# BolinLai/CSTS

Hardware: AMD Instinct MI355X
Metric: clips/sec training (fwd+bwd) CSTS-Ego4D 16x256^2 bf16 (higher is better)
Workload: dtype bf16; 1 GPU; CSTS_Ego4D_Gaze_Forecast.yaml train step (fwd + KLDiv + 0.05*EgoNCE + bwd + clip + AdamW), 16x256^2 video + 24 kHz STFT audio, b=4/GPU; mode=train, global_batch=4, frames=16, crop=256, parallelism=dp1, step=hip_graph, hip_graph=True, rccl_ranks=1

## Files before the change

### csts_amd/csrc/attention.hip

```cpp
#include <type_traits>
#include <utility>
#include "common.h"

#ifndef CSTS_ATTN_PART
#define CSTS_ATTN_PART 0
#endif
#ifndef CSTS_DKV_DEPTH
#define CSTS_DKV_DEPTH 4
#endif
#ifndef CSTS_DKV_SWZ
#define CSTS_DKV_SWZ 0
#endif

#ifdef CSTS_ATTN_STAMPS
#if CSTS_ATTN_PART == 1
__device__ unsigned long long g_attn_stamps[4096];
#else
static __device__ unsigned long long g_attn_stamps[4096];
#endif
#define AT_STAMP() do { if (stamp_on && nstamp < 4000) g_attn_stamps[nstamp++] = (unsigned long long)__builtin_amdgcn_s_memtime(); } while (0)
#if CSTS_ATTN_PART == 1
extern "C" int csts_debug_attn_stamps(unsigned long long* dst_host) {
  return (int)hipMemcpyFromSymbol(dst_host, HIP_SYMBOL(g_attn_stamps), sizeof(unsigned long long) * 4096);
}
// ... 863 lines not shown

  tile_loop_dma<HD, KBLK, LD, false>(smem, p.K, kbase, p.k_ts, p.V, vbase, p.v_ts, 0, p.Nk, tid,
                                     [&](const bf16* Ks, const bf16* Vs, int) {
    constexpr int NS = HD / 16, ND = HD / 32, SCB = 2 * NS, PVB = 2 * ND, DEPTH = 4, NBLK = 2 * KT, TOTAL = KT * (SCB + PVB);
    typedef __attribute__((address_space(3))) s16x4 lds_s16x4;
    const int g1 = (lane >> 4) & 1, qq = (lane & 15) >> 2, pp = lane & 3;
    const bf16* rowK = Ks + (lane & 31) * LD + 8 * h;
    const bf16* rowV = Vs + (lane & 31) * LD + 8 * h;
    const bf16* trK = Ks + (4 * h + qq) * LD + 16 * g1 + 4 * pp;
    auto blk_pv = [](int bi) constexpr { return bi == NBLK - 1 || (bi >= 2 && (bi & 1) == 0); };
    auto blk_unit = [](int bi) constexpr { return bi == 0 ? 0 : bi == NBLK - 1 ? KT - 1 : (bi & 1) ? (bi + 1) / 2 : bi / 2 - 1; };
    auto blk_of = [=](int g) constexpr { int bi = 0, s0 = 0; for (;; ++bi) { const int n = blk_pv(bi) ? PVB : SCB; if (g < s0 + n) return bi; s0 += n; } };
    auto blk_start = [=](int bi) constexpr { int s0 = 0; for (int i = 0; i < bi; ++i) s0 += blk_pv(i) ? PVB : SCB; return s0; };
    bf16x8 ring[DEPTH + 1];
    auto request = [&](auto gc) {
      constexpr int g = decltype(gc)::value, bi = blk_of(g), u = blk_unit(bi), k = g - blk_start(bi);
      bf16x8& dst = ring[g % (DEPTH + 1)];
      if constexpr (!blk_pv(bi)) {
        dst = *reinterpret_cast<const bf16x8*>((k < NS ? rowK : rowV) + u * 32 * LD + 16 * (k % NS));
      } else {
        constexpr int s2 = k / ND, d = k % ND;
        const bf16* Yb = trK + (u * 32 + 16 * s2) * LD + 32 * d;
        const bf16x4 b0 = __builtin_bit_cast(bf16x4, __builtin_amdgcn_ds_read_tr16_b64_v4i16((lds_s16x4*)(Yb)));
        const bf16x4 b1 = __builtin_bit_cast(bf16x4, __builtin_amdgcn_ds_read_tr16_b64_v4i16((lds_s16x4*)(Yb + 8 * LD)));
        dst[0] = b0[0]; dst[1] = b0[1]; dst[2] = b0[2]; dst[3] = b0[3];
        dst[4] = b1[0]; dst[5] = b1[1]; dst[6] = b1[2]; dst[7] = b1[3];
      }
    };
    static_for<DEPTH>([&](auto gc) { request(gc); });
    f32x16 S[2], dP[2];
    bf16x8 bp[2][2];
    auto piece = [&](auto suc, auto qc) {
      constexpr int sp = decltype(suc)::value & 1, q = decltype(qc)::value;
#pragma unroll
      for (int r = 2 * q; r < 2 * q + 2; ++r) {
        const float ds = __builtin_amdgcn_exp2f(__builtin_fmaf(S[sp][r], p.scale_log2, negL)) * (dP[sp][r] - dl);
        bp[sp][r / 8][r % 8] = (bf16)ds;
      }
    };
    static_for<TOTAL>([&](auto gc) {
      constexpr int g = decltype(gc)::value, bi = blk_of(g), u = blk_unit(bi), k = g - blk_start(bi), par = u & 1;
      constexpr bool is_pv = blk_pv(bi);
      if constexpr (!is_pv && k == 0) {
#pragma unroll
        for (int r = 0; r < 16; ++r) { S[par][r] = 0.f; dP[par][r] = 0.f; }
      }
      if constexpr (g + DEPTH < TOTAL) request(std::integral_constant<int, g + DEPTH>{});
      const bf16x8 a = ring[g % (DEPTH + 1)];
      if constexpr (!is_pv) {
        if constexpr (k < NS) S[par] = CSTS_MFMA16(a, qf.b[k], S[par], 0, 0, 0);
        else dP[par] = CSTS_MFMA16(a, dof.b[k - NS], dP[par], 0, 0, 0);
      } else {
        constexpr int s2 = k / ND, d = k % ND;
        acc[d] = CSTS_MFMA16(a, bp[par][s2], acc[d], 0, 0, 0);
      }
      if constexpr (bi == 1) {
        if constexpr (k < 8) piece(std::integral_constant<int, 0>{}, std::integral_constant<int, k>{});
      } else if constexpr (bi >= 2 && (bi & 1) == 0) {
        constexpr int su = bi / 2;
        if constexpr (k < 4) piece(std::integral_constant<int, su>{}, std::integral_constant<int, k>{});
        else {
          piece(std::integral_constant<int, su>{}, std::integral_constant<int, 4 + 2 * (k - 4)>{});
          piece(std::integral_constant<int, su>{}, std::integral_constant<int, 5 + 2 * (k - 4)>{});
        }
      }
      __builtin_amdgcn_sched_barrier(0);
    });
  });
  stage_rows_out<HD>(smem, p.dQ, (int64_t)b * p.dq_bs + (int64_t)head * p.dq_hs, p.dq_ts, BX * 128, p.Nq, acc, p.scale,
                     w * 32 + (lane & 31), h, tid);
}

template <int HD, bool F32, bool SLOW>
__global__ __launch_bounds__(256) void attn_dkv_kernel(AttnP p) {
  typedef typename El<F32>::T T;
  typedef Cfg<HD, F32> C;
  constexpr bool FAST = !F32 && HD == 96 && !SLOW;
  constexpr bool SWZ = FAST && (CSTS_DKV_SWZ != 0);
  constexpr int LDF = SWZ ? 128 : C::LD_ROW;
  constexpr int QBLK = FAST ? 128 : C::KVBLK, QT = QBLK / 32;
  extern __shared__ __attribute__((aligned(16))) char smem_raw[];
  T* smem = reinterpret_cast<T*>(smem_raw);
  const int tid = threadIdx.x, lane = tid & 63, w = tid >> 6, h = lane >> 5;
  int BX, BY, BZ;
  xcd_remap3(BX, BY, BZ);
  const int b = BZ / p.H, head = BZ % p.H;
  const int split = BY;
  const int kraw = BX * 128 + w * 32 + (lane & 31);
  const bool kvalid = kraw < p.Nk;
  const int ki = kvalid ? kraw : p.Nk - 1;

  RowFrag<HD, F32> kf, vf;
  kf.load(p.K, (int64_t)b * p.k_bs + (int64_t)ki * p.k_ts + (int64_t)head * p.k_hs, h);
  vf.load(p.V, (int64_t)b * p.v_bs + (int64_t)ki * p.v_ts + (int64_t)head * p.v_hs, h);
  f32x16 dK[HD / 32], dV[HD / 32];
#pragma unroll
  for (int d = 0; d < HD / 32; ++d)
#pragma unroll
    for (int r = 0; r < 16; ++r) { dK[d][r] = 0.f; dV[d][r] = 0.f; }
  const int64_t qbase = (int64_t)b * p.q_bs + (int64_t)head * p.q_hs;
  const int64_t dobase = (int64_t)b * p.do_bs + (int64_t)head * p.do_hs;
  const int qbeg = split * p.q_chunk, qend = min(p.Nq, qbeg + p.q_chunk);
  const float* Lrow = p.LSE + ((int64_t)b * p.H + head) * p.Nq;
  const float* Drow = p.delta + ((int64_t)b * p.H + head) * p.Nq;
  const int fk = frame_of(p, ki);
#ifdef CSTS_ATTN_STAMPS
  const bool stamp_on = tid == 0 && BX == 0 && BY == 0 && BZ == 0;
  int nstamp = 1;
  const unsigned long long rt0 = (unsigned long long)__builtin_amdgcn_s_memrealtime();
#endif
  AT_STAMP();

  auto tile_body = [&](const T* Qs, const T* dOs, int q0, const float* Ls, auto&& dma) {
    const float* Ds = Ls + QBLK;
    AT_STAMP();
    auto softmax_bwd = [&](f32x16& S, f32x16& dP, int qt, int r0, int n) {
      const int j = r0 >> 2, qo = qt * 32 + 8 * j + 4 * h;
      const float4 L4 = *reinterpret_cast<const float4*>(Ls + qo), D4 = *reinterpret_cast<const float4*>(Ds + qo);
      const float l[4] = {L4.x, L4.y, L4.z, L4.w}, dd[4] = {D4.x, D4.y, D4.z, D4.w};
#pragma unroll
      for (int r = r0; r < r0 + n; ++r) {
        const int i = r & 3;
        const float e = __builtin_amdgcn_exp2f(__builtin_fmaf(S[r], p.scale_log2, -l[i]));
        float pr = e;
        if constexpr (SLOW) {
          const int q = q0 + qo + i;
          const bool dead = (q >= qend) | ((p.mask_mode != 0) & (frame_of(p, q) != fk));
          pr = dead ? 0.f : e;
        }
        S[r] = pr;
        dP[r] = pr * (dP[r] - dd[i]);
      }
    };
    if constexpr (F32 || HD != 96) {
#pragma unroll
      for (int qt = 0; qt < QT; ++qt) {
        f32x16 S, dP;
#pragma unroll
        for (int r = 0; r < 16; ++r) { S[r] = 0.f; dP[r] = 0.f; }
        score<HD, C::LD_ROW, F32>(S, Qs + qt * 32 * C::LD_ROW, kf, lane);
        score<HD, C::LD_ROW, F32>(dP, dOs + qt * 32 * C::LD_ROW, vf, lane);
#pragma unroll
        for (int j = 0; j < 4; ++j) softmax_bwd(S, dP, qt, 4 * j, 4);
        pv<HD, C::LD_ROW, F32>(dV, dOs + qt * 32 * C::LD_ROW, S, lane);
        pv<HD, C::LD_ROW, F32>(dK, Qs + qt * 32 * C::LD_ROW, dP, lane);
      }
    } else {
      constexpr int LD = LDF, NS = HD / 16, ND = HD / 32, BLK = 2 * NS, DEPTH = CSTS_DKV_DEPTH, NBLK = 2 * QT, TOTAL = BLK * NBLK;
      static_assert(BLK == 4 * ND, "S/dP and dV/dK blocks have the same number of slots");
      static_assert(QT >= 2, "the block order needs two units");
      typedef __attribute__((address_space(3))) s16x4 lds_s16x4;
      const int g1 = (lane >> 4) & 1, qq = (lane & 15) >> 2, pp = lane & 3;
      constexpr int DOFF = QBLK * LD;
      int rowo[NS], tro[ND][2];
#pragma unroll
      for (int k = 0; k < NS; ++k)
        rowo[k] = (lane & 31) * LD + (SWZ ? (((2 * k + h) ^ swz16(lane & 15)) * 8) : (16 * k + 8 * h));
#pragma unroll
      for (int d = 0; d < ND; ++d)
#pragma unroll
        for (int rd = 0; rd < 2; ++rd) {
          const int row = 4 * h + qq + 8 * rd;
          tro[d][rd] = row * LD + (SWZ ? ((((4 * d + 2 * g1 + (pp >> 1)) ^ swz16(row)) * 8) + 4 * (pp & 1)) : (32 * d + 16 * g1 + 4 * pp));
        }
      bf16x8 ring[DEPTH + 1];
      auto blk_pv = [](int bi) constexpr { return bi == NBLK - 1 || (bi >= 2 && (bi & 1) == 0); };
      auto blk_unit = [](int bi) constexpr { return bi == 0 ? 0 : bi == NBLK - 1 ? QT - 1 : (bi & 1) ? (bi + 1) / 2 : bi / 2 - 1; };
      auto hp_slot = [](int u, int j) constexpr {
        const int w0 = (u == 0 ? BLK : u == QT - 1 ? BLK * (NBLK - 2) : BLK * 2 * u) + 1;
        const int n = ((u == 0 || u == QT - 1) ? BLK : 2 * BLK) - 1;
        return w0 + j * n / 16;
      };
      auto request = [&](auto gc) {
        constexpr int g = decltype(gc)::value, bi = g / BLK, k = g % BLK;
        constexpr bool is_pv = blk_pv(bi);
        constexpr int u = blk_unit(bi);
        bf16x8& dst = ring[g % (DEPTH + 1)];
        if constexpr (!is_pv) {
          dst = *reinterpret_cast<const bf16x8*>(Qs + rowo[k % NS] + (k < NS ? 0 : DOFF) + u * 32 * LD);
        } else {
          constexpr int idx = k % (2 * ND), s2 = idx / ND, d = idx % ND;
          const bf16* Yb = Qs + (k < 2 * ND ? DOFF : 0) + (u * 32 + 16 * s2) * LD;
          const bf16x4 b0 = __builtin_bit_cast(bf16x4, __builtin_amdgcn_ds_read_tr16_b64_v4i16((lds_s16x4*)(Yb + tro[d][0])));
          const bf16x4 b1 = __builtin_bit_cast(bf16x4, __builtin_amdgcn_ds_read_tr16_b64_v4i16((lds_s16x4*)(Yb + tro[d][1])));
          dst[0] = b0[0]; dst[1] = b0[1]; dst[2] = b0[2]; dst[3] = b0[3];
          dst[4] = b1[0]; dst[5] = b1[1]; dst[6] = b1[2]; dst[7] = b1[3];
        }
      };
      static_for<DEPTH>([&](auto gc) { request(gc); });
      f32x16 S[2], dP[2];
      bf16x8 bpS[2][2], bpD[2][2];
      float4 Lq[2][4], Dq[2][4];
      auto comp = [](const float4& v, int i) { return i == 0 ? v.x : i == 1 ? v.y : i == 2 ? v.z : v.w; };
      auto half_piece = [&](auto uc, auto jc) {
        constexpr int u = decltype(uc)::value, j = decltype(jc)::value, sp = u & 1, r0 = 2 * (j / 2), quad = r0 >> 2;
        if constexpr ((j & 1) == 0) {
#pragma unroll
          for (int r = r0; r < r0 + 2; ++r) {
            float e = __builtin_amdgcn_exp2f(__builtin_fmaf(S[sp][r], p.scale_log2, -comp(Lq[sp][quad], r & 3)));
            if constexpr (SLOW) {
              const int q = q0 + u * 32 + 8 * quad + 4 * h + (r & 3);
              const bool dead = (q >= qend) | ((p.mask_mode != 0) & (frame_of(p, q) != fk));
              e = dead ? 0.f : e;
            }
            S[sp][r] = e;
          }
        } else {
#pragma unroll
          for (int r = r0; r < r0 + 2; ++r) dP[sp][r] = S[sp][r] * (dP[sp][r] - comp(Dq[sp][quad], r & 3));
          constexpr int s2 = r0 / 8, e0 = r0 % 8;
          bpS[sp][s2][e0] = (bf16)S[sp][r0]; bpS[sp][s2][e0 + 1] = (bf16)S[sp][r0 + 1];
          bpD[sp][s2][e0] = (bf16)dP[sp][r0]; bpD[sp][s2][e0 + 1] = (bf16)dP[sp][r0 + 1];
        }
      };
      constexpr int NDMA = tile_dma_count<QBLK, LD>();
      static_for<TOTAL>([&](auto gc) {
        constexpr int g = decltype(gc)::value, bi = g / BLK, k = g % BLK;
        constexpr bool is_pv = blk_pv(bi);
        constexpr int u = blk_unit(bi), par = u & 1;
        if constexpr (k == 0) { AT_STAMP(); }
        if constexpr (!is_pv && k == 0) {
#pragma unroll
          for (int r = 0; r < 16; ++r) { S[par][r] = 0.f; dP[par][r] = 0.f; }
        }
        if constexpr (!is_pv && k < 8) {
          const int qo = u * 32 + 8 * (k & 3) + 4 * h;
          if constexpr (k < 4) Lq[par][k] = *reinterpret_cast<const float4*>(Ls + qo);
          else Dq[par][k - 4] = *reinterpret_cast<const float4*>(Ds + qo);
        }
#ifndef CSTS_DKV_DIAG_NOREAD
        if constexpr (g + DEPTH < TOTAL) request(std::integral_constant<int, g + DEPTH>{});
#endif
        const bf16x8 a = ring[g % (DEPTH + 1)];
        if constexpr (!is_pv) {
          if constexpr (k < NS) S[par] = CSTS_MFMA16(a, kf.b[k], S[par], 0, 0, 0);
          else dP[par] = CSTS_MFMA16(a, vf.b[k - NS], dP[par], 0, 0, 0);
        } else {
          constexpr int idx = k % (2 * ND), s2 = idx / ND, d = idx % ND;
#if defined(CSTS_DKV_DIAG_BFRAG) || defined(CSTS_DKV_DIAG_BZERO)
          asm volatile("" ::"v"(bpS[par][s2]), "v"(bpD[par][s2]));
#endif
#ifdef CSTS_DKV_DIAG_BFRAG
          if constexpr (k < 2 * ND) dV[d] = CSTS_MFMA16(a, kf.b[s2 + 2 * par], dV[d], 0, 0, 0);
          else dK[d] = CSTS_MFMA16(a, vf.b[s2 + 2 * par], dK[d], 0, 0, 0);
#elif defined(CSTS_DKV_DIAG_BZERO)
          bf16x8 zz;
#pragma unroll
          for (int e = 0; e < 8; ++e) zz[e] = (bf16)0.f;
          asm volatile("" : "+v"(zz));
          if constexpr (k < 2 * ND) dV[d] = CSTS_MFMA16(a, zz, dV[d], 0, 0, 0);
          else dK[d] = CSTS_MFMA16(a, zz, dK[d], 0, 0, 0);
#else
          if constexpr (k < 2 * ND) dV[d] = CSTS_MFMA16(a, bpS[par][s2], dV[d], 0, 0, 0);
          else dK[d] = CSTS_MFMA16(a, bpD[par][s2], dK[d], 0, 0, 0);
#endif
        }
#ifdef CSTS_DKV_DIAG_NOSM
        if constexpr (!is_pv && k == BLK - 1) asm volatile("" ::"v"(S[par]), "v"(dP[par]));
#endif
#ifndef CSTS_DKV_DIAG_NOSM
        static_for<QT * 16>([&](auto ic) {
          constexpr int i = decltype(ic)::value, su = i / 16, j = i % 16;
          if constexpr (hp_slot(su, j) == g) half_piece(std::integral_constant<int, su>{}, std::integral_constant<int, j>{});
        });
#endif
#ifndef CSTS_DKV_DIAG_NODMA
        if constexpr (g < NDMA) dma(std::integral_constant<int, g>{});
#endif
        __builtin_amdgcn_sched_barrier(0);
      });
    }
    AT_STAMP();
  };
  if constexpr (FAST)
    tile_loop_dma<HD, QBLK, LDF, true, LDF, true, SWZ>(smem, p.Q, qbase, p.q_ts, p.dO, dobase, p.do_ts, qbeg, qend, tid, tile_body,
                                                       Lrow, Drow AT_STAMP_ARGS);
  else
    tile_loop<HD, QBLK, C::LD_ROW, C::LD_ROW, F32, true>(smem, p.Q, qbase, p.q_ts, p.dO, dobase, p.do_ts, qbeg, qend, tid,
                                                         [&](const T* Qs, const T* dOs, int q0, const float* Ls) {
                                                           tile_body(Qs, dOs, q0, Ls, [](auto) {});
                                                         }, Lrow, Drow AT_STAMP_ARGS);
  AT_STAMP();
#ifdef CSTS_ATTN_STAMPS
  if (stamp_on) {
    g_attn_stamps[0] = nstamp;
    g_attn_stamps[4095] = (unsigned long long)__builtin_amdgcn_s_memrealtime() - rt0;
  }
#endif
  if (!kvalid) return;
  if (p.nsplit == 1) {
    store_rows<HD>(p.dK, p.dt, (int64_t)b * p.dk_bs + (int64_t)ki * p.dk_ts + (int64_t)head * p.dk_hs, dK, p.scale, h);
    store_rows<HD>(p.dV, p.dt, (int64_t)b * p.dv_bs + (int64_t)ki * p.dv_ts + (int64_t)head * p.dv_hs, dV, 1.f, h);
  } else {
    const int64_t per = (int64_t)p.B * p.H * p.Nk * HD;
    const int64_t off = (((int64_t)split * p.B + b) * p.H + head) * (int64_t)p.Nk * HD + (int64_t)ki * HD;
    store_rows<HD>(p.ws, CSTS_F32, off, dK, p.scale, h);
    store_rows<HD>(p.ws, CSTS_F32, (int64_t)p.nsplit * per + off, dV, 1.f, h);
  }
}

template <int HD>
__global__ __launch_bounds__(256) void attn_bwd_fused_kernel(AttnP p) {
  typedef Cfg<HD, false> C;
  constexpr int LD = C::LD_ROW, TILE = 128 * LD;
  __shared__ __attribute__((aligned(16))) bf16 smem[5 * TILE + 512];
  bf16* Ks = smem;
  bf16* Vs = smem + TILE;
  bf16* Qs = smem + 2 * TILE;
  bf16* dOs = smem + 3 * TILE;
  bf16* Os = smem + 4 * TILE;
  float* Ls = reinterpret_cast<float*>(smem + 5 * TILE);
  float* Ds = Ls + 128;
  const int tid = threadIdx.x, lane = tid & 63, w = tid >> 6, h = lane >> 5;
  int BX, BY, BZ;
  xcd_remap3(BX, BY, BZ);
  const int b = BY / p.H, head = BY % p.H;
  const int split = BX;
  const int qbeg = split * p.q_chunk, qend = min(p.Nq, qbeg + p.q_chunk);
  const int64_t kbase = (int64_t)b * p.k_bs + (int64_t)head * p.k_hs, vbase = (int64_t)b * p.v_bs + (int64_t)head * p.v_hs;
  const int64_t qbase = (int64_t)b * p.q_bs + (int64_t)head * p.q_hs, dobase = (int64_t)b * p.do_bs + (int64_t)head * p.do_hs;
  const int64_t obase = (int64_t)b * p.o_bs + (int64_t)head * p.o_hs;
  {
    TileStage<HD, 128> sk, sv;
    sk.gload(p.K, kbase, p.k_ts, 0, p.Nk, tid);
    sv.gload(p.V, vbase, p.v_ts, 0, p.Nk, tid);
    sk.lstore(Ks, LD, tid);
    sv.lstore(Vs, LD, tid);
  }

  const int kraw = w * 32 + (lane & 31);
  const bool kvalid = kraw < p.Nk;
  const int ki = kvalid ? kraw : p.Nk - 1;
  RowFrag<HD, false> kf, vf;
  kf.load(p.K, kbase + (int64_t)ki * p.k_ts, h);
  vf.load(p.V, vbase + (int64_t)ki * p.v_ts, h);
  f32x16 dK[HD / 32], dV[HD / 32];
#pragma unroll
  for (int d = 0; d < HD / 32; ++d)
#pragma unroll
    for (int r = 0; r < 16; ++r) { dK[d][r] = 0.f; dV[d][r] = 0.f; }
  const float* Lrow = p.LSE + ((int64_t)b * p.H + head) * p.Nq;

  TileStage<HD, 128> sq, sdo, so;
  float lnext = 0.f;
  sq.gload(p.Q, qbase, p.q_ts, qbeg, qend, tid);
  sdo.gload(p.dO, dobase, p.do_ts, qbeg, qend, tid);
  so.gload(p.O, obase, p.o_ts, qbeg, qend, tid);
  if (tid < 128) lnext = Lrow[min(qbeg + tid, qend - 1)];
  for (int q0 = qbeg; q0 < qend; q0 += 128) {
    __syncthreads();
    sq.lstore(Qs, LD, tid);
    sdo.lstore(dOs, LD, tid);
    so.lstore(Os, LD, tid);
    if (tid < 128) Ls[tid] = lnext;
    if (q0 + 128 < qend) {
      sq.gload(p.Q, qbase, p.q_ts, q0 + 128, qend, tid);
      sdo.gload(p.dO, dobase, p.do_ts, q0 + 128, qend, tid);
      so.gload(p.O, obase, p.o_ts, q0 + 128, qend, tid);
      if (tid < 128) lnext = Lrow[min(q0 + 128 + tid, qend - 1)];
    }
    __syncthreads();
    f32x16 acc[HD / 32];
#pragma unroll
    for (int d = 0; d < HD / 32; ++d)
#pragma unroll
      for (int r = 0; r < 16; ++r) acc[d][r] = 0.f;
    {
      const int qrow = w * 32 + (lane & 31);
      RowFrag<HD, false> qf, dof;
      frag_from_lds<HD>(qf, Qs, qrow, h);
      frag_from_lds<HD>(dof, dOs, qrow, h);
      float dl = 0.f;
      {
        RowFrag<HD, false> of;
        frag_from_lds<HD>(of, Os, qrow, h);
#pragma unroll
        for (int s2 = 0; s2 < HD / 16; ++s2)
#pragma unroll
          for (int j2 = 0; j2 < 8; ++j2) dl += (float)dof.b[s2][j2] * (float)of.b[s2][j2];
      }
      dl += __shfl_xor(dl, 32, 64);
      if (h == 0) Ds[qrow] = dl;
      const float negL = -Ls[qrow];
#pragma unroll
      for (int kt = 0; kt < 4; ++kt) {
        if (kt * 32 >= p.Nk) break;
        f32x16 S, dP;
#pragma unroll
        for (int r = 0; r < 16; ++r) { S[r] = 0.f; dP[r] = 0.f; }
        score<HD, LD, false>(S, Ks + kt * 32 * LD, qf, lane);
        score<HD, LD, false>(dP, Vs + kt * 32 * LD, dof, lane);
#pragma unroll
        for (int r = 0; r < 16; ++r) {
          const float e = __builtin_amdgcn_exp2f(__builtin_fmaf(S[r], p.scale_log2, negL));
          const float pr = (kt * 32 + rowoff(r, h) >= p.Nk) ? 0.f : e;
          S[r] = pr * (dP[r] - dl);
        }
        pv<HD, LD, false>(acc, Ks + kt * 32 * LD, S, lane);
      }
    }
    stage_rows_out_wave<HD>(Os, p.dQ, (int64_t)b * p.dq_bs + (int64_t)head * p.dq_hs, p.dq_ts, q0, qend, acc, p.scale, w, lane);
    __syncthreads();
    const bool ragged = q0 + 128 > qend;
#pragma unroll
    for (int qt = 0; qt < 4; ++qt) {
      f32x16 S, dP;
#pragma unroll
      for (int r = 0; r < 16; ++r) { S[r] = 0.f; dP[r] = 0.f; }
      score<HD, LD, false>(S, Qs + qt * 32 * LD, kf, lane);
      score<HD, LD, false>(dP, dOs + qt * 32 * LD, vf, lane);
#pragma unroll
      for (int j = 0; j < 4; ++j) {
        const int qo = qt * 32 + 8 * j + 4 * h;
        const float4 L4 = *reinterpret_cast<const float4*>(Ls + qo), D4 = *reinterpret_cast<const float4*>(Ds + qo);
        const float l[4] = {L4.x, L4.y, L4.z, L4.w}, dd[4] = {D4.x, D4.y, D4.z, D4.w};
#pragma unroll
        for (int i = 0; i < 4; ++i) {
          const float e = __builtin_amdgcn_exp2f(__builtin_fmaf(S[4 * j + i], p.scale_log2, -l[i]));
          const float pr = (ragged && q0 + qo + i >= qend) ? 0.f : e;
          S[4 * j + i] = pr;
          dP[4 * j + i] = pr * (dP[4 * j + i] - dd[i]);
        }
      }
      pv<HD, LD, false>(dV, dOs + qt * 32 * LD, S, lane);
      pv<HD, LD, false>(dK, Qs + qt * 32 * LD, dP, lane);
    }
  }
  if (!kvalid) return;
  if (p.nsplit == 1) {
    store_rows<HD>(p.dK, p.dt, (int64_t)b * p.dk_bs + (int64_t)ki * p.dk_ts + (int64_t)head * p.dk_hs, dK, p.scale, h);
    store_rows<HD>(p.dV, p.dt, (int64_t)b * p.dv_bs + (int64_t)ki * p.dv_ts + (int64_t)head * p.dv_hs, dV, 1.f, h);
  } else {
    const int64_t per = (int64_t)p.B * p.H * p.Nk * HD;
    const int64_t off = (((int64_t)split * p.B + b) * p.H + head) * (int64_t)p.Nk * HD + (int64_t)ki * HD;
    store_rows<HD>(p.ws, CSTS_F32, off, dK, p.scale, h);
    store_rows<HD>(p.ws, CSTS_F32, (int64_t)p.nsplit * per + off, dV, 1.f, h);
  }
}

#if CSTS_ATTN_PART == 0
__global__ __launch_bounds__(256) void attn_dkv_reduce_kernel(AttnP p, int HD) {
  const int64_t per = (int64_t)p.B * p.H * p.Nk * HD;
  const int H8 = HD / 8;
  const int64_t total8 = 2 * per / 8;
  for (int64_t i8 = (int64_t)blockIdx.x * blockDim.x + threadIdx.x; i8 < total8; i8 += (int64_t)gridDim.x * blockDim.x) {
    const int64_t idx = i8 * 8;
    const int which = idx >= per;
    int64_t e = idx - which * per;
    float s[8] = {0.f, 0.f, 0.f, 0.f, 0.f, 0.f, 0.f, 0.f};
    for (int sp = 0; sp < p.nsplit; ++sp) {
      const float4* q = reinterpret_cast<const float4*>(p.ws + ((int64_t)which * p.nsplit + sp) * per + e);
      const float4 a = q[0], b4 = q[1];
      s[0] += a.x; s[1] += a.y; s[2] += a.z; s[3] += a.w; s[4] += b4.x; s[5] += b4.y; s[6] += b4.z; s[7] += b4.w;
    }
    int64_t r = e / 8;
    const int d = (int)(r % H8) * 8; r /= H8;
    const int k = (int)(r % p.Nk); r /= p.Nk;
    const int head = (int)(r % p.H);
    const int b = (int)(r / p.H);
    if (which == 0) st8_from_f32(p.dK, p.dt, (int64_t)b * p.dk_bs + (int64_t)k * p.dk_ts + (int64_t)head * p.dk_hs + d, s);
    else st8_from_f32(p.dV, p.dt, (int64_t)b * p.dv_bs + (int64_t)k * p.dv_ts + (int64_t)head * p.dv_hs + d, s);
  }
}

__global__ __launch_bounds__(256) void attn_probs_kernel(AttnP p, int HD, float* probs) {
  const int64_t total = (int64_t)p.B * p.H * p.Nq * p.Nk;
  for (int64_t idx = (int64_t)blockIdx.x * blockDim.x + threadIdx.x; idx < total; idx += (int64_t)gridDim.x * blockDim.x) {
    const int k = (int)(idx % p.Nk);
    int64_t e = idx / p.Nk;
    const int q = (int)(e % p.Nq); e /= p.Nq;
    const int head = (int)(e % p.H);
    const int b = (int)(e / p.H);
    float s = 0.f;
    const int64_t qo = (int64_t)b * p.q_bs + (int64_t)q * p.q_ts + (int64_t)head * p.q_hs;
    const int64_t ko = (int64_t)b * p.k_bs + (int64_t)k * p.k_ts + (int64_t)head * p.k_hs;
    for (int d = 0; d < HD; ++d) s += ld_as_f32(p.Q, p.dt, qo + d) * ld_as_f32(p.K, p.dt, ko + d);
    const float L = p.LSE[((int64_t)b * p.H + head) * p.Nq + q];
    probs[idx] = is_masked(p, q, k) ? 0.f : exp2f(s * p.scale_log2 - L);
  }
}

#endif
#if CSTS_ATTN_PART == 0
template <int HD, bool F32> size_t smem_fwd() {
  typedef Cfg<HD, F32> C;
  return (size_t)C::KVBLK * (C::LD_ROW + C::LD_TR) * (F32 ? 4 : 2 * 2);
}
template <int HD, bool F32> size_t smem_bwd() {
  typedef Cfg<HD, F32> C;
  return (size_t)C::KVBLK * 2 * C::LD_ROW * (F32 ? 4 : 2 * 2);
}

int fill(const csts_attn_args* a, AttnP& p) {
  p.Q = a->Q; p.K = a->K; p.V = a->V; p.O = a->O; p.LSE = a->LSE; p.dO = a->dO; p.delta = a->delta;
  p.dQ = a->dQ; p.dK = a->dK; p.dV = a->dV; p.ws = nullptr;
  p.dt = a->dtype; p.B = a->B; p.H = a->H; p.Nq = a->Nq; p.Nk = a->Nk;
  p.q_bs = a->q_strides[0]; p.q_ts = a->q_strides[1]; p.q_hs = a->q_strides[2];
  p.k_bs = a->k_strides[0]; p.k_ts = a->k_strides[1]; p.k_hs = a->k_strides[2];
  p.v_bs = a->v_strides[0]; p.v_ts = a->v_strides[1]; p.v_hs = a->v_strides[2];
  p.o_bs = a->o_strides[0]; p.o_ts = a->o_strides[1]; p.o_hs = a->o_strides[2];
  p.do_bs = a->do_strides[0]; p.do_ts = a->do_strides[1]; p.do_hs = a->do_strides[2];
  p.dq_bs = a->dq_strides[0]; p.dq_ts = a->dq_strides[1]; p.dq_hs = a->dq_strides[2];
  p.dk_bs = a->dk_strides[0]; p.dk_ts = a->dk_strides[1]; p.dk_hs = a->dk_strides[2];
  p.dv_bs = a->dv_strides[0]; p.dv_ts = a->dv_strides[1]; p.dv_hs = a->dv_strides[2];
  p.scale = a->scale;
  p.scale_log2 = a->scale * 1.4426950408889634f;
  p.mask_mode = a->mask_mode; p.mask_T = a->mask_T; p.mask_HW = a->mask_HW;
  p.mask_inv_hw = (a->mask_mode != 0 && a->mask_HW > 0) ? 1.f / (float)a->mask_HW : 0.f;
  p.q_chunk = 0; p.nsplit = 1;
  return 0;
}

bool strides_ok(const int64_t* s, int dt) {
  const int a = dt == CSTS_F32 ? 4 : 8;
  return s[0] % a == 0 && s[1] % a == 0 && s[2] % a == 0;
}

struct AttnSwitches { bool fwd_fast, dkv_fast, fused; int dq; };
const AttnSwitches& attn_switches() {
  static const AttnSwitches s = [] {
    auto num = [](const char* name) { const char* e = getenv(name); return e ? atoi(e) : -1; };
    return AttnSwitches{num("CSTS_ATTN_FWD_FAST") != 0, num("CSTS_ATTN_DKV_FAST") != 0, num("CSTS_ATTN_FUSED_BWD") != 0, num("CSTS_ATTN_DQ_FAST")};
  }();
  return s;
}

enum { FWD_GENERIC, FWD_FAST };
enum { DQ_NONE, DQ_GENERIC, DQ_FAST64, DQ_FAST128 };
enum { DKV_ONE_PASS, DKV_FAST, DKV_SLOW, DKV_PLAIN };
struct AttnRoute { int fwd, dq, dkv, nsplit, q_chunk; size_t ws_bytes; };

bool attn_route(const csts_attn_args* a, AttnRoute* r) {
  if (!a || a->B <= 0 || a->H <= 0 || a->Nq <= 0 || a->Nk <= 0 || (a->head_dim != 96 && a->head_dim != 192)) return false;
  const AttnSwitches& sw = attn_switches();
  const int Nq = a->Nq, Nk = a->Nk, hd = a->head_dim;
  const bool h16 = a->dtype == CSTS_BF16, open = a->mask_mode == 0;
  const bool fast96 = h16 && hd == 96 && open;
  r->fwd = sw.fwd_fast && fast96 && Nk % 64 == 0 ? FWD_FAST : FWD_GENERIC;
  int qblk;
  int64_t want;
  if (sw.fused && fast96 && Nk <= 128 && Nq >= 1024) {
    r->dq = DQ_NONE; r->dkv = DKV_ONE_PASS; qblk = 128;
    want = std::max<int64_t>(1, std::min<int64_t>(256 / ((int64_t)a->B * a->H), cdiv(Nq, 256)));
  } else {
    if (sw.dq == 0 || !fast96 || Nk % 64 != 0) r->dq = DQ_GENERIC;
    else r->dq = (sw.dq == 4 && Nk % 128 == 0) ? DQ_FAST128 : DQ_FAST64;
    if (sw.dkv_fast && fast96 && Nq % 128 == 0) r->dkv = DKV_FAST;
    else r->dkv = (h16 && hd == 192 && open && Nq % 32 == 0) ? DKV_PLAIN : DKV_SLOW;
    qblk = r->dkv == DKV_FAST ? 128 : hd == 96 ? 64 : 32;
    want = std::max<int64_t>(1, 256 / (cdiv(Nk, 128) * a->B * a->H));
    want = std::max<int64_t>(1, std::min<int64_t>(want, cdiv(Nq, 4 * qblk)));
  }
  r->q_chunk = (int)(cdiv(cdiv(Nq, want), qblk) * qblk);
  r->nsplit = (int)cdiv(Nq, r->q_chunk);
  r->ws_bytes = r->nsplit > 1 ? (size_t)2 * r->nsplit * a->B * a->H * Nk * hd * sizeof(float) : 16;
  return true;
}

}

#define ATTN_COMMON_CHECKS(a)                                                                           \
  CSTS_REQUIRE((a) != nullptr, "null args");                                                            \
  CSTS_REQUIRE((a)->head_dim == 96 || (a)->head_dim == 192, "head_dim must be 96 or 192");              \
  CSTS_REQUIRE((a)->dtype == CSTS_F32 || (a)->dtype == CSTS_BF16, "bad dtype");                         \
  CSTS_REQUIRE((a)->B > 0 && (a)->H > 0 && (a)->Nq > 0 && (a)->Nk > 0, "empty problem");                \
  CSTS_REQUIRE((a)->Q && (a)->K && (a)->V, "null q/k/v");                                               \
  CSTS_REQUIRE(aligned16((a)->Q) && aligned16((a)->K) && aligned16((a)->V), "q/k/v must be 16-byte aligned"); \
  CSTS_REQUIRE(strides_ok((a)->q_strides, (a)->dtype) && strides_ok((a)->k_strides, (a)->dtype) &&      \
                   strides_ok((a)->v_strides, (a)->dtype),                                             \
               "strides must keep 16-byte row alignment");                                              \
  if ((a)->mask_mode == CSTS_MASK_SPATIAL)                                                              \
  CSTS_REQUIRE((a)->mask_HW > 0 && (a)->Nq < (1 << 20) && (a)->Nq == (a)->mask_T * (a)->mask_HW + (a)->mask_T && (a)->Nk == (a)->Nq, "spatial mask needs Nq == Nk == T*HW + T < 2^20")

template <int HD, bool F32>
static bool launch_fwd(const AttnRoute& r, const AttnP& p, dim3 grid, hipStream_t stream) {
  const size_t sm = smem_fwd<HD, F32>();
  if (r.fwd == FWD_FAST) hipLaunchKernelGGL(attn_fwd_fast_kernel, grid, dim3(256), sm, stream, p);
  else hipLaunchKernelGGL((attn_fwd_kernel<HD, F32>), grid, dim3(256), sm, stream, p);
  return true;
}
template <int HD, bool F32>
static bool launch_dq(const AttnRoute& r, const AttnP& p, dim3 grid, hipStream_t stream) {
  const size_t sm = smem_bwd<HD, F32>();
  if (r.dq == DQ_FAST128) {
    constexpr size_t sm4 = (size_t)2 * 128 * 2 * Cfg<96, false>::LD_ROW * 2;
    if (!csts_dyn_lds_optin(reinterpret_cast<const void*>(&attn_dq_fast_kernel<4>), (int)sm4)) return false;
    hipLaunchKernelGGL(attn_dq_fast_kernel<4>, grid, dim3(256), sm4, stream, p);
  } else if (r.dq == DQ_FAST64) hipLaunchKernelGGL(attn_dq_fast_kernel<2>, grid, dim3(256), sm, stream, p);
  else hipLaunchKernelGGL((attn_dq_kernel<HD, F32>), grid, dim3(256), sm, stream, p);
  return true;
}
template <int HD, bool F32>
static bool launch_dkv(const AttnRoute& r, const AttnP& p, dim3 grid, hipStream_t stream) {
  const size_t sm = smem_bwd<HD, F32>() + (size_t)Cfg<HD, F32>::KVBLK * 4 * sizeof(float);
  if (r.dkv == DKV_FAST) return csts_attn_dkv_fast_launch(p, grid, stream);
  if constexpr (HD == 192 && !F32) {
    if (r.dkv == DKV_PLAIN) {
      hipLaunchKernelGGL((attn_dkv_kernel<192, false, false>), grid, dim3(256), sm, stream, p);
      return true;
    }
  }
  hipLaunchKernelGGL((attn_dkv_kernel<HD, F32, true>), grid, dim3(256), sm, stream, p);
  return true;
}
#define LAUNCH_BY_TYPE(fn, a, ...)                                                                                   \
  ((a)->head_dim == 96 ? ((a)->dtype == CSTS_F32 ? fn<96, true>(__VA_ARGS__) : fn<96, false>(__VA_ARGS__))           \
                       : ((a)->dtype == CSTS_F32 ? fn<192, true>(__VA_ARGS__) : fn<192, false>(__VA_ARGS__)))

static void launch_reduce(const csts_attn_args* a, const AttnP& p, hipStream_t stream) {
  const int64_t total = (int64_t)2 * a->B * a->H * a->Nk * a->head_dim / 8;
  hipLaunchKernelGGL(attn_dkv_reduce_kernel, dim3((unsigned)std::min<int64_t>(cdiv(total, 256), 4096)), dim3(256), 0, stream, p,
                     a->head_dim);
}

extern "C" int csts_attn_fwd(const csts_attn_args* a, hipStream_t stream) {
  ATTN_COMMON_CHECKS(a);
  CSTS_REQUIRE(a->O && a->LSE && aligned16(a->O) && strides_ok(a->o_strides, a->dtype), "bad output");
  AttnP p; fill(a, p);
  AttnRoute r;
  CSTS_REQUIRE(attn_route(a, &r), "no route");
  dim3 grid((unsigned)cdiv(a->Nq, 128), a->H, a->B);
  CSTS_REQUIRE(LAUNCH_BY_TYPE(launch_fwd, a, r, p, grid, stream), "hipFuncSetAttribute(MaxDynamicSharedMemorySize) failed on this device");
  CSTS_LAUNCH_CHECK();
  return 0;
}

extern "C" size_t csts_attn_bwd_workspace(const csts_attn_args* a) {
  AttnRoute r;
  return attn_route(a, &r) ? r.ws_bytes : 0;
}

extern "C" int csts_attn_route(const csts_attn_args* a, char* buf, int buflen, int* nsplit, int* q_chunk) {
  CSTS_REQUIRE(buf != nullptr && buflen > 0 && nsplit != nullptr && q_chunk != nullptr, "null pointer");
  AttnRoute r;
  CSTS_REQUIRE(attn_route(a, &r), "no route: null args, empty problem, or head_dim not 96 / 192");
  *nsplit = r.nsplit;
  *q_chunk = r.q_chunk;
  const int hd = a->head_dim;
  const char* t = a->dtype == CSTS_BF16 ? "false" : "true";
  char fwd[48] = "attn_fwd_fast_kernel", dq[48] = "", dkv[48] = "attn_bwd_fused_kernel";
  if (r.fwd == FWD_GENERIC) snprintf(fwd, sizeof fwd, "attn_fwd_kernel<%d,%s>", hd, t);
  if (r.dq == DQ_GENERIC) snprintf(dq, sizeof dq, "attn_dq_kernel<%d,%s>", hd, t);
  else if (r.dq != DQ_NONE) snprintf(dq, sizeof dq, "attn_dq_fast_kernel<%d>", r.dq == DQ_FAST128 ? 4 : 2);
  if (r.dkv == DKV_SLOW) snprintf(dkv, sizeof dkv, "attn_dkv_kernel<%d,%s,true>", hd, t);
  else if (r.dkv != DKV_ONE_PASS) snprintf(dkv, sizeof dkv, "attn_dkv_kernel<%d,false,false>", hd);
  const int n = snprintf(buf, buflen, "%s;%s;%s;%s", fwd, dq, dkv, r.nsplit > 1 ? "attn_dkv_reduce_kernel" : "");
  CSTS_REQUIRE(n < buflen, "buffer too small");
  return 0;
}

extern "C" int csts_attn_bwd(const csts_attn_args* a, void* workspace, size_t ws_bytes, hipStream_t stream) {
  ATTN_COMMON_CHECKS(a);
  CSTS_REQUIRE(a->O && a->LSE && a->dO && a->delta && a->dQ && a->dK && a->dV, "null backward operand");
  CSTS_REQUIRE(aligned16(a->dO) && aligned16(a->dQ) && aligned16(a->dK) && aligned16(a->dV), "alignment");
  CSTS_REQUIRE(strides_ok(a->do_strides, a->dtype) && strides_ok(a->dq_strides, a->dtype) &&
                   strides_ok(a->dk_strides, a->dtype) && strides_ok(a->dv_strides, a->dtype) &&
                   strides_ok(a->o_strides, a->dtype), "strides must keep 16-byte row alignment");
  AttnP p; fill(a, p);
  AttnRoute r;
  CSTS_REQUIRE(attn_route(a, &r), "no route");
  p.nsplit = r.nsplit; p.q_chunk = r.q_chunk;
  if (r.nsplit > 1) {
    if (workspace == nullptr || ws_bytes < r.ws_bytes) CSTS_FAIL("workspace too small [workspace != nullptr && ws_bytes >= csts_attn_bwd_workspace(a)]");
    p.ws = reinterpret_cast<float*>(workspace);
  }
  if (r.dkv == DKV_ONE_PASS) {
    hipLaunchKernelGGL((attn_bwd_fused_kernel<96>), dim3((unsigned)p.nsplit, (unsigned)(a->B * a->H)), dim3(256), 0, stream, p);
  } else {
    dim3 grid_dq((unsigned)cdiv(a->Nq, 128), a->H, a->B);
    CSTS_REQUIRE(LAUNCH_BY_TYPE(launch_dq, a, r, p, grid_dq, stream), "hipFuncSetAttribute(MaxDynamicSharedMemorySize) failed on this device");
    CSTS_LAUNCH_CHECK();
    dim3 grid_dkv((unsigned)cdiv(a->Nk, 128), p.nsplit, a->B * a->H);
    CSTS_REQUIRE(LAUNCH_BY_TYPE(launch_dkv, a, r, p, grid_dkv, stream), "hipFuncSetAttribute(MaxDynamicSharedMemorySize) failed on this device");
  }
  CSTS_LAUNCH_CHECK();
  if (r.nsplit > 1) {
    launch_reduce(a, p, stream);
    CSTS_LAUNCH_CHECK();
  }
  return 0;
}

extern "C" int csts_attn_probs(const csts_attn_args* a, float* probs, hipStream_t stream) {
  ATTN_COMMON_CHECKS(a);
  CSTS_REQUIRE(a->LSE && probs, "null pointer");
  AttnP p; fill(a, p);
  const int64_t total = (int64_t)a->B * a->H * a->Nq * a->Nk;
  hipLaunchKernelGGL(attn_probs_kernel, dim3((unsigned)std::min<int64_t>(cdiv(total, 256), 4096)), dim3(256), 0, stream, p,
                     a->head_dim, probs);
  CSTS_LAUNCH_CHECK();
  return 0;
}
#else
}
bool csts_attn_dkv_fast_launch(const csts_attn::AttnP& p, dim3 grid, hipStream_t stream) {
  constexpr size_t smf = (size_t)2 * 128 * 2 * (CSTS_DKV_SWZ ? 128 : Cfg<96, false>::LD_ROW) * 2 + 2 * 2 * 128 * sizeof(float);
  if (!csts_dyn_lds_optin(reinterpret_cast<const void*>(&attn_dkv_kernel<96, false, false>), (int)smf)) return false;
  hipLaunchKernelGGL((attn_dkv_kernel<96, false, false>), grid, dim3(256), smf, stream, p);
  return true;
}
#endif
```

Before: 210.5 clips/s.

## Reuse dS from dK/dV pass for dQ via LDS instead of recomputing scores

The fused attention backward kernel used to compute dQ by recomputing QK^T and dO·V^T scores and the softmax per query row before the dK/dV pass. Now the dK/dV pass writes bf16 dS into an LDS tile that reuses the O tile's space. After a barrier, dQ = dS·K is computed with transposed LDS reads (ds_read_tr16) feeding MFMA. This removes two score GEMMs and the exponentials per tile. In exchange it adds LDS traffic, an extra barrier and a larger LDS footprint. dS is also rounded to bf16 before the dQ product, which can change numerics.

```diff
diff --git a/csts_amd/csrc/attention.hip b/csts_amd/csrc/attention.hip
--- a/csts_amd/csrc/attention.hip
+++ b/csts_amd/csrc/attention.hip
@@ -1189,14 +1189,19 @@
 template <int HD>
 __global__ __launch_bounds__(256) void attn_bwd_fused_kernel(AttnP p) {
   typedef Cfg<HD, false> C;
+  typedef __attribute__((address_space(3))) s16x4 lds_s16x4;
   constexpr int LD = C::LD_ROW, TILE = 128 * LD;
-  __shared__ __attribute__((aligned(16))) bf16 smem[5 * TILE + 512];
+  constexpr int LDD = 156, DTILE = 128 * LDD;
+  static_assert(DTILE >= TILE && LDD % 4 == 0 && LDD >= 128, "the dS tile takes the O tile's place; 8-byte aligned rows");
+  __shared__ __attribute__((aligned(16))) bf16 smem[4 * TILE + DTILE + 512];
+  static_assert(sizeof(bf16) * (4 * TILE + DTILE + 512) <= 160 * 1024, "one workgroup's LDS");
   bf16* Ks = smem;
   bf16* Vs = smem + TILE;
   bf16* Qs = smem + 2 * TILE;
   bf16* dOs = smem + 3 * TILE;
   bf16* Os = smem + 4 * TILE;
-  float* Ls = reinterpret_cast<float*>(smem + 5 * TILE);
+  bf16* dSs = Os;
+  float* Ls = reinterpret_cast<float*>(smem + 4 * TILE + DTILE);
   float* Ds = Ls + 128;
   const int tid = threadIdx.x, lane = tid & 63, w = tid >> 6, h = lane >> 5;
   int BX, BY, BZ;
@@ -1218,6 +1223,7 @@
   const int kraw = w * 32 + (lane & 31);
   const bool kvalid = kraw < p.Nk;
   const int ki = kvalid ? kraw : p.Nk - 1;
+  const unsigned kmask = kvalid ? 0xffffffffu : 0u;
   RowFrag<HD, false> kf, vf;
   kf.load(p.K, kbase + (int64_t)ki * p.k_ts, h);
   vf.load(p.V, vbase + (int64_t)ki * p.v_ts, h);
@@ -1227,6 +1233,11 @@
 #pragma unroll
     for (int r = 0; r < 16; ++r) { dK[d][r] = 0.f; dV[d][r] = 0.f; }
   const float* Lrow = p.LSE + ((int64_t)b * p.H + head) * p.Nq;
+  const int trk = 4 * h + ((lane & 15) >> 2), trc = 16 * ((lane >> 4) & 1) + 4 * (lane & 3);
+  const bf16* Ktr = Ks + trk * LD + trc;
+  const bf16* dStr = dSs + trk * LDD + 32 * w + trc;
+  bf16* dSrow = dSs + kraw * LDD + 4 * h;
+  const int nkt = min(4, (p.Nk + 31) >> 5);
 
   TileStage<HD, 128> sq, sdo, so;
   float lnext = 0.f;
@@ -1247,46 +1258,19 @@
       if (tid < 128) lnext = Lrow[min(q0 + 128 + tid, qend - 1)];
     }
     __syncthreads();
-    f32x16 acc[HD / 32];
-#pragma unroll
-    for (int d = 0; d < HD / 32; ++d)
-#pragma unroll
-      for (int r = 0; r < 16; ++r) acc[d][r] = 0.f;
     {
       const int qrow = w * 32 + (lane & 31);
-      RowFrag<HD, false> qf, dof;
-      frag_from_lds<HD>(qf, Qs, qrow, h);
+      RowFrag<HD, false> dof, of;
       frag_from_lds<HD>(dof, dOs, qrow, h);
+      frag_from_lds<HD>(of, Os, qrow, h);
       float dl = 0.f;
-      {
-        RowFrag<HD, false> of;
-        frag_from_lds<HD>(of, Os, qrow, h);
-#pragma unroll
-        for (int s2 = 0; s2 < HD / 16; ++s2)
-#pragma unroll
-          for (int j2 = 0; j2 < 8; ++j2) dl += (float)dof.b[s2][j2] * (float)of.b[s2][j2];
-      }
+#pragma unroll
+      for (int s2 = 0; s2 < HD / 16; ++s2)
+#pragma unroll
+        for (int j2 = 0; j2 < 8; ++j2) dl += (float)dof.b[s2][j2] * (float)of.b[s2][j2];
       dl += __shfl_xor(dl, 32, 64);
       if (h == 0) Ds[qrow] = dl;
-      const float negL = -Ls[qrow];
-#pragma unroll
-      for (int kt = 0; kt < 4; ++kt) {
-        if (kt * 32 >= p.Nk) break;
-        f32x16 S, dP;
-#pragma unroll
-        for (int r = 0; r < 16; ++r) { S[r] = 0.f; dP[r] = 0.f; }
-        score<HD, LD, false>(S, Ks + kt * 32 * LD, qf, lane);
-        score<HD, LD, false>(dP, Vs + kt * 32 * LD, dof, lane);
-#pragma unroll
-        for (int r = 0; r < 16; ++r) {
-          const float e = __builtin_amdgcn_exp2f(__builtin_fmaf(S[r], p.scale_log2, negL));
-          const float pr = (kt * 32 + rowoff(r, h) >= p.Nk) ? 0.f : e;
-          S[r] = pr * (dP[r] - dl);
-        }
-        pv<HD, LD, false>(acc, Ks + kt * 32 * LD, S, lane);
-      }
-    }
-    stage_rows_out_wave<HD>(Os, p.dQ, (int64_t)b * p.dq_bs + (int64_t)head * p.dq_hs, p.dq_ts, q0, qend, acc, p.scale, w, lane);
+    }
     __syncthreads();
     const bool ragged = q0 + 128 > qend;
 #pragma unroll
@@ -1301,17 +1285,59 @@
         const int qo = qt * 32 + 8 * j + 4 * h;
         const float4 L4 = *reinterpret_cast<const float4*>(Ls + qo), D4 = *reinterpret_cast<const float4*>(Ds + qo);
         const float l[4] = {L4.x, L4.y, L4.z, L4.w}, dd[4] = {D4.x, D4.y, D4.z, D4.w};
+        bf16x4 ds4;
 #pragma unroll
         for (int i = 0; i < 4; ++i) {
           const float e = __builtin_amdgcn_exp2f(__builtin_fmaf(S[4 * j + i], p.scale_log2, -l[i]));
           const float pr = (ragged && q0 + qo + i >= qend) ? 0.f : e;
           S[4 * j + i] = pr;
           dP[4 * j + i] = pr * (dP[4 * j + i] - dd[i]);
+          ds4[i] = (bf16)dP[4 * j + i];
         }
+        uint2 u = __builtin_bit_cast(uint2, ds4);
+        u.x &= kmask; u.y &= kmask;
+        *reinterpret_cast<uint2*>(dSrow + qt * 32 + 8 * j) = u;
       }
       pv<HD, LD, false>(dV, dOs + qt * 32 * LD, S, lane);
       pv<HD, LD, false>(dK, Qs + qt * 32 * LD, dP, lane);
     }
+    __syncthreads();
+    f32x16 acc[HD / 32];
+#pragma unroll
+    for (int d = 0; d < HD / 32; ++d)
+#pragma unroll
+      for (int r = 0; r < 16; ++r) acc[d][r] = 0.f;
+#pragma unroll
+    for (int kt = 0; kt < 4; ++kt) {
+      if (kt >= nkt) break;
+      s16x4 kt4[2][HD / 32][2], ds4[2][2];
+#pragma unroll
+      for (int s = 0; s < 2; ++s) {
+        ds4[s][0] = __builtin_amdgcn_ds_read_tr16_b64_v4i16((lds_s16x4*)(dStr + (kt * 32 + 16 * s) * LDD));
+        ds4[s][1] = __builtin_amdgcn_ds_read_tr16_b64_v4i16((lds_s16x4*)(dStr + (kt * 32 + 16 * s + 8) * LDD));
+#pragma unroll
+        for (int d = 0; d < HD / 32; ++d) {
+          kt4[s][d][0] = __builtin_amdgcn_ds_read_tr16_b64_v4i16((lds_s16x4*)(Ktr + (kt * 32 + 16 * s) * LD + 32 * d));
+          kt4[s][d][1] = __builtin_amdgcn_ds_read_tr16_b64_v4i16((lds_s16x4*)(Ktr + (kt * 32 + 16 * s + 8) * LD + 32 * d));
+        }
+      }
+#pragma unroll
+      for (int s = 0; s < 2; ++s) {
+        const bf16x4 p0 = __builtin_bit_cast(bf16x4, ds4[s][0]), p1 = __builtin_bit_cast(bf16x4, ds4[s][1]);
+        bf16x8 bp;
+        bp[0] = p0[0]; bp[1] = p0[1]; bp[2] = p0[2]; bp[3] = p0[3];
+        bp[4] = p1[0]; bp[5] = p1[1]; bp[6] = p1[2]; bp[7] = p1[3];
+#pragma unroll
+        for (int d = 0; d < HD / 32; ++d) {
+          const bf16x4 b0 = __builtin_bit_cast(bf16x4, kt4[s][d][0]), b1 = __builtin_bit_cast(bf16x4, kt4[s][d][1]);
+          bf16x8 a;
+          a[0] = b0[0]; a[1] = b0[1]; a[2] = b0[2]; a[3] = b0[3];
+          a[4] = b1[0]; a[5] = b1[1]; a[6] = b1[2]; a[7] = b1[3];
+          acc[d] = CSTS_MFMA16(a, bp, acc[d], 0, 0, 0);
+        }
+      }
+    }
+    stage_rows_out_wave<HD>(Qs, p.dQ, (int64_t)b * p.dq_bs + (int64_t)head * p.dq_hs, p.dq_ts, q0, qend, acc, p.scale, w, lane);
   }
   if (!kvalid) return;
   if (p.nsplit == 1) {
```

New measurement: 211.3 clips/s, median of 6. Within noise of the previous version (+0.4%).
